# GiulioRomualdi/paper_romualdi_2022_icra_centroidal-mpc-walking

Measured on AMD Instinct MI355X. Metric: centroidal-MPC solves/sec (batch, horizon=20), higher is better.
Workload: dtype f32

## Files before the change

### paper_romualdi_2022_icra_centroidal-mpc-walking_amd/csrc/cmpc_solver.hip

```cpp
#include "cmpc_device.h"
#include "cmpc_launch.h"

#include <cstdlib>
#include <type_traits>
#include <map>
#include <mutex>

#define NS CMPC_NS
#define NF CMPC_NF
#define NQ CMPC_NQ
#define NU CMPC_NU
#define NXA CMPC_NXA
#define NI CMPC_NI
#define PLD 39
#define GLD 30
#define RLD 36
#define NPAN 46
#define GEO 36
#define SQ_TILE_WAVES 6
#define SQ_SPIN_MAX (1 << 20)
#define SQ_PUB_FLOATS (10 * NPAN * 4 + 128 * 4)
#define ZLD 36
#define MSET (NU * RLD + NPAN * RLD + NS * 16)
#define NTRI 256
// ... 16 lines not shown
#define PROF_DECL long long pt_ = __builtin_amdgcn_s_memtime()
#define PROF(slot) do { long long n_ = __builtin_amdgcn_s_memtime(); if (threadIdx.x == 0 && blockIdx.x == 0) g_prof[slot] += n_ - pt_; pt_ = n_; } while (0)
#define PROF2_DECL long long pt2_ = __builtin_amdgcn_s_memtime()
#define PROF3(slot) do { long long n_ = __builtin_amdgcn_s_memtime(); if (threadIdx.x == 192 && blockIdx.x == 0) g_prof[slot] += n_ - pt2_; pt2_ = n_; } while (0)
#define PROF4(slot) do { long long n_ = __builtin_amdgcn_s_memtime(); if (threadIdx.x == 128 && blockIdx.x == 0) g_prof[slot] += n_ - pt2_; pt2_ = n_; } while (0)
#define PROF2(slot) do { long long n_ = __builtin_amdgcn_s_memtime(); if (threadIdx.x == 0 && blockIdx.x == 0) g_prof[slot] += n_ - pt2_; pt2_ = n_; } while (0)
#define PROF5(slot) do { long long n_ = __builtin_amdgcn_s_memtime(); if (threadIdx.x == 216 && blockIdx.x == 0) g_prof[slot] += n_ - pt2_; pt2_ = n_; } while (0)
#define CPROF(i) do { if (ln == 0 && blockIdx.x == 0 && k < N) atomicAdd(reinterpret_cast<unsigned long long*>(&g_prof[32 + 5 * wv + (i)]), (unsigned long long)(__builtin_amdgcn_s_memtime() - pc0_)); } while (0)
#define CPROF2(i) do { if (ln == 0 && blockIdx.x == 0 && k < N) atomicAdd(reinterpret_cast<unsigned long long*>(&g_prof[64 + 8 * wv + (i)]), (unsigned long long)(__builtin_amdgcn_s_memtime() - pc0_)); } while (0)
#ifdef CMPC_PROFILE_LIGHT
#undef PROF2_DECL
#undef PROF2
#undef PROF3
#undef PROF4
#undef PROF5
#undef CPROF
#undef CPROF2
#define CPROF2(i)
#define PROF2_DECL
#define PROF2(slot)
#define PROF3(slot)
#define PROF4(slot)
#define PROF5(slot)
#define CPROF(i)
#define SQPROF_DECL
#define SQPROF(slot)
#else
#define SQPROF_DECL PROF_DECL
#define SQPROF(slot) PROF(slot)
#endif
#else
#define SQPROF_DECL
#define SQPROF(slot)
#define CPROF(i)
#define CPROF2(i)
#define PROF_DECL
#define PROF(slot)
#define PROF2_DECL
#define PROF2(slot)
#define PROF3(slot)
#define PROF4(slot)
#define PROF5(slot)
#endif

struct Ctx {
    CmpcIdx L;
    int N;
    const float* sp;
    float *S, *U, *T, *Z;
    float* LAM;
    float *dS, *dU, *dT, *dZ, *d;
    float *Lf;
    float *geoA;
    float *P0, *Qb, *G, *QuuF, *Pan, *Bval, *Aval, *arow, *ybuf, *fpv, *fpn;
    float *idstrip;
    float *ZT;
    double *QuuD1, *qs1;
    int *Brow, *Arow, *qmask;
    unsigned short* tri;
    double *QuuD, *pv, *pn, *qs, *Pd, *sig, *gco, *redd;
    float* red;
    int* flag;
    int* prog;
};

__device__ inline void wave_lds_sync() { asm volatile("" ::: "memory"); }
typedef __attribute__((address_space(3))) const float* ldsf_t;
typedef __attribute__((address_space(3))) float* ldsw_t;
__device__ inline ldsf_t lds_opaque(const float* p) { ldsf_t q = (ldsf_t)p; asm volatile("" : "+v"(q)); return q; }
__device__ inline ldsw_t lds_opaque_w(float* p) { ldsw_t q = (ldsw_t)p; asm volatile("" : "+v"(q)); return q; }
__device__ inline ldsf_t lds_opaque_again(ldsf_t q) { asm volatile("" : "+v"(q)); return q; }
typedef float v4f __attribute__((ext_vector_type(4)));
typedef float v2f __attribute__((ext_vector_type(2)));
__device__ inline float4 lds_ld4(ldsf_t p)
{
    const v4f v = *reinterpret_cast<__attribute__((address_space(3))) const v4f*>(p);
    return make_float4(v[0], v[1], v[2], v[3]);
}
__device__ inline void lds_ld4x4(ldsf_t p, float4 (&out)[4])
{
    v4f a, b, c, d;
    asm volatile("ds_read_b128 %0, %4\n\tds_read_b128 %1, %4 offset:16\n\tds_read_b128 %2, %4 offset:32\n\tds_read_b128 %3, %4 offset:48\n\ts_waitcnt lgkmcnt(0)"
                 : "=&v"(a), "=&v"(b), "=&v"(c), "=&v"(d)
                 : "v"(p)
                 : "memory");
    out[0] = make_float4(a[0], a[1], a[2], a[3]);
    out[1] = make_float4(b[0], b[1], b[2], b[3]);
    out[2] = make_float4(c[0], c[1], c[2], c[3]);
    out[3] = make_float4(d[0], d[1], d[2], d[3]);
}

typedef unsigned v4u __attribute__((ext_vector_type(4)));
template <bool G>
struct RecRef;
template <>
struct RecRef<false> {
    float* p;
    __device__ RecRef(float* base, int, int k) : p(base + (size_t)REC_N * k) {}
    __device__ float ld(unsigned off) const { return p[off]; }
    __device__ float4 ld4(unsigned off) const { return *reinterpret_cast<const float4*>(p + off); }
    __device__ void st(unsigned off, float v) const { p[off] = v; }
    __device__ void st4(unsigned off, const float4& w) const { *reinterpret_cast<float4*>(p + off) = w; }
};
template <>
struct RecRef<true> {
    typedef __attribute__((address_space(1))) unsigned gu32_t;
    typedef __attribute__((address_space(1))) v4u gv4u_t;
    __amdgpu_buffer_rsrc_t r;
    unsigned so;
    char* gb;
    __device__ RecRef(float* base, int N, int k)
    {
        const unsigned long long a = (unsigned long long)base;
        const unsigned lo = __builtin_amdgcn_readfirstlane((unsigned)a), hi = __builtin_amdgcn_readfirstlane((unsigned)(a >> 32));
// ... 7 lines not shown
        const v4u v = __builtin_amdgcn_raw_buffer_load_b128(r, 4u * off, so, 0);
        return make_float4(__uint_as_float(v.x), __uint_as_float(v.y), __uint_as_float(v.z), __uint_as_float(v.w));
    }
    __device__ void st(unsigned off, float v) const { *(gu32_t*)(gb + 4u * off) = __float_as_uint(v); }
    __device__ void st4(unsigned off, const float4& w) const
    {
        const v4u v = {__float_as_uint(w.x), __float_as_uint(w.y), __float_as_uint(w.z), __float_as_uint(w.w)};
        *(gv4u_t*)(gb + 4u * off) = v;
    }
};

template <bool FG>
__device__ inline void make_ctx(Ctx& c, char* smem, int N, float* fg_base)
{
    constexpr int KBYTES = (sizeof(CmpcConsts) + 15) & ~15;
    c.L.N = N;
    c.N = N;
    double* dp = reinterpret_cast<double*>(smem + KBYTES);
    c.QuuD = dp; dp += 90;
    c.pv = dp; dp += 40; c.pn = dp; dp += 40; c.qs = dp; dp += 16; c.Pd = dp; dp += 40;
    c.sig = dp; dp += NI; c.gco = dp; dp += NI; dp += 2 * NI;
    c.redd = dp; dp += 8;
    c.QuuD1 = c.QuuD; c.qs1 = c.qs;
    if (!FG) { c.QuuD1 = dp; dp += 90; c.qs1 = dp; dp += 16; }
    float* fp = reinterpret_cast<float*>(dp);
    c.QuuF = fp; fp += NU * RLD;
    c.Pan = fp; fp += NPAN * RLD;
    c.ZT = nullptr;
    if (!FG) {
        c.G = nullptr; c.P0 = nullptr;
        c.Qb = fp; fp += NS * 16;
        fp += MSET;
        c.ZT = fp; fp += SQ_PUB_FLOATS;
    } else {
    c.G = fp; fp += (NXA * GLD + 3) & ~3;
    c.P0 = fp; fp += (NXA * PLD + 3) & ~3; c.Qb = fp; fp += NS * 16;
    }
    {
        float* vp = c.QuuF;
        c.dS = vp; vp += NS * (N + 1); c.dU = vp; vp += NU * N; c.dT = vp; vp += NI * N; c.dZ = vp;
    }
    c.ybuf = fp; fp += 96;
    c.idstrip = fp; fp += ID_STRIPS;
    if (!FG) { c.Lf = fp; fp += (size_t)REC_N * N; } else c.Lf = fg_base;
    c.sp = fp; fp += (c.L.np() + 3) & ~3;
    c.S = fp; fp += NS * (N + 1); c.U = fp; fp += NU * N;
    if (!FG || N <= CMPC_TZ_LDS_NMAX) { c.T = fp; fp += NI * N; c.Z = fp; fp += NI * N; }
    else { c.T = fg_base + (size_t)REC_N * N; c.Z = c.T + NI * N; }
    c.d = fp; fp += NS * N;
    c.LAM = fp; fp += NS * (N + 1);
    c.geoA = fp; fp += GEO * N;
    c.Bval = fp; fp += 3 * NU; c.Aval = fp; fp += 3 * NS + 3;
    c.arow = fp; fp += 96 + 12; fp += DSET_F;
    c.fpv = fp; fp += 40; c.fpn = fp; fp += 40; c.red = fp; fp += 24;
    c.Brow = reinterpret_cast<int*>(fp); fp += 3 * NU;
    c.Arow = reinterpret_cast<int*>(fp); fp += 3 * NS + 3; fp += DSET_I;
    c.flag = reinterpret_cast<int*>(fp); fp += 4;
    c.prog = c.flag;
    if (!FG) { c.prog = reinterpret_cast<int*>(fp); fp += 128; }
    c.qmask = reinterpret_cast<int*>(fp); fp += CMPC_NMAX;
    c.tri = reinterpret_cast<unsigned short*>(fp); fp += NTRI / 2;
}

__device__ inline void use_desc_set(Ctx& c, int s)
{
    c.Bval += s * DSET_F; c.Aval += s * DSET_F; c.arow += s * DSET_F;
    c.Brow += s * DSET_I; c.Arow += s * DSET_I;
    c.sig += s * 2 * NI; c.gco += s * 2 * NI;
}

__device__ inline int ub_row(int m) { const int I = m >> 2; return REC_UB + 16 * (8 * I - I * (I - 1) / 2) + (m & 3) * 4 * (8 - I); }
__device__ inline int wt_idx(int j, int a) { return REC_WT + 32 * j + 4 * ((a >> 2) ^ (j & 7)) + (a & 3); }
__device__ inline float half_sum(float v)
{
    const auto r = __builtin_amdgcn_permlane32_swap(__float_as_uint(v), __float_as_uint(v), false, false);
    return __uint_as_float(r[0]) + __uint_as_float(r[1]);
}
__device__ inline float oct_sum(float v)
{
    v += __uint_as_float(__builtin_amdgcn_update_dpp(0u, __float_as_uint(v), 0xB1, 0xF, 0xF, true));
    v += __uint_as_float(__builtin_amdgcn_update_dpp(0u, __float_as_uint(v), 0x4E, 0xF, 0xF, true));
    v += __uint_as_float(__builtin_amdgcn_update_dpp(0u, __float_as_uint(v), 0x141, 0xF, 0xF, true));
    return v;
}
__device__ inline float dot4(const float4& a, const float4& b) { return a.x * b.x + a.y * b.y + a.z * b.z + a.w * b.w; }

__device__ inline float gam_of(const Ctx& c, int ct, int k) { return c.sp[c.L.pGam(ct) + k]; }
__device__ inline float Rm(const float* R, int r, int cc) { return R[3 * cc + r]; }

__device__ inline bool qfree_compute(const Ctx& c, int k, int m)
{
    const int ct = m / 3, i = m % 3;
    const float lo = c.sp[c.L.pLo(ct) + 3 * k + i], hi = c.sp[c.L.pUp(ct) + 3 * k + i];
    return gam_of(c, ct, k) < 0.5f && (hi - lo) > 1e-9f;
}
__device__ inline bool qfree(const Ctx& c, int k, int m) { return (c.qmask[k] >> m) & 1; }
__device__ inline bool outside_subset(const Ctx& c, int ct, int k)
{
    const float g = gam_of(c, ct, k);
    if (g == 0.f) return false;
    if (g != 1.f) return true;
    int kp = -1;
    for (int j = k - 1; j >= 0 && kp < 0; --j) if (gam_of(c, ct, j) < 0.5f) kp = j;
    const float* R = c.sp + c.L.pR(ct) + 9 * k;
    const float* nom = c.sp + c.L.pNom(ct) + 3 * (k + 1);
    const float* lo = c.sp + c.L.pLo(ct) + 3 * k;
    const float* up = c.sp + c.L.pUp(ct) + 3 * k;
// ... 127 lines not shown
}

__device__ inline double grad_sym(const Ctx& c, const CmpcConsts& prm, int k, int m)
{
    const int ct = m / 12, i = m % 3;
    const float* u = c.U + NU * k + 12 * ct;
    const double gam = gam_of(c, ct, k);
    const double mean = 0.25 * ((double)u[i] + (double)u[3 + i] + (double)u[6 + i] + (double)u[9 + i]);
    const double esum = 4.0 * mean * (1.0 - gam);
    const double e = (double)c.U[NU * k + m] - gam * mean;
    return 2.0 * prm.w_sym * (e - 0.25 * gam * esum);
}

__device__ inline float readlane_f(float x, int lane) { return __int_as_float(__builtin_amdgcn_readlane(__float_as_int(x), lane)); }
__device__ inline float uniform_f(float x) { return __int_as_float(__builtin_amdgcn_readfirstlane(__float_as_int(x))); }
__device__ inline double uniform_d(double x)
{
    return __hiloint2double(__builtin_amdgcn_readfirstlane(__double2hiint(x)), __builtin_amdgcn_readfirstlane(__double2loint(x)));
}
__device__ inline double readlane_d(double x, int lane)
{
    const int lo = __builtin_amdgcn_readlane(__double2loint(x), lane);
    const int hi = __builtin_amdgcn_readlane(__double2hiint(x), lane);
    return __hiloint2double(hi, lo);
}

template <int CTRL>
__device__ inline float dpp_f(float v) { return __uint_as_float(__builtin_amdgcn_update_dpp(0u, __float_as_uint(v), CTRL, 0xF, 0xF, true)); }
template <int CTRL>
__device__ inline double dpp_d(double v)
{
    const int lo = __builtin_amdgcn_update_dpp(0, __double2loint(v), CTRL, 0xF, 0xF, true);
    const int hi = __builtin_amdgcn_update_dpp(0, __double2hiint(v), CTRL, 0xF, 0xF, true);
    return __hiloint2double(hi, lo);
}
__device__ inline float amax_nan(float m, float v) { return (v == v) ? fmaxf(m, fabsf(v)) : INFINITY; }
__device__ inline float row_target(float z, float mu_min) { return fmaxf(mu_min * fminf(1.f, z * z), 1e-4f * mu_min); }
__device__ inline float wave_max(float v)
{
    v = fmaxf(v, dpp_f<0xB1>(v));
    v = fmaxf(v, dpp_f<0x4E>(v));
    v = fmaxf(v, dpp_f<0x141>(v));
    v = fmaxf(v, dpp_f<0x140>(v));
    return fmaxf(fmaxf(readlane_f(v, 0), readlane_f(v, 16)), fmaxf(readlane_f(v, 32), readlane_f(v, 48)));
}
__device__ inline double wave_sum(double v)
{
    v += dpp_d<0xB1>(v);
    v += dpp_d<0x4E>(v);
    v += dpp_d<0x141>(v);
    v += dpp_d<0x140>(v);
    return (readlane_d(v, 0) + readlane_d(v, 16)) + (readlane_d(v, 32) + readlane_d(v, 48));
}
template <int NT, int NV>
__device__ inline void block_maxn(float (&v)[NV], float* red, int tid)
{
#pragma unroll
    for (int q = 0; q < NV; ++q) v[q] = wave_max(v[q]);
    __syncthreads();
    if ((tid & 63) == 0) {
#pragma unroll
        for (int q = 0; q < NV; ++q) red[3 * (tid >> 6) + q] = v[q];
    }
    __syncthreads();
#pragma unroll
    for (int q = 0; q < NV; ++q) {
        float r = red[q];
#pragma unroll
        for (int w = 1; w < NT / 64; ++w) r = fmaxf(r, red[3 * w + q]);
        v[q] = uniform_f(r);
    }
}
template <int NT>
__device__ inline double block_sum(double v, double* red, int tid)
{
    v = wave_sum(v);
    __syncthreads();
    if ((tid & 63) == 0) red[tid >> 6] = v;
    __syncthreads();
    double r = red[0];
#pragma unroll
    for (int w = 1; w < NT / 64; ++w) r += red[w];
    return uniform_d(r);
}
template <int NT>
__device__ inline void block_max2_sum(float& m0, float& m1, double& sm, float* red, double* redd, int tid)
{
    m0 = wave_max(m0); m1 = wave_max(m1); sm = wave_sum(sm);
    __syncthreads();
    if ((tid & 63) == 0) { red[3 * (tid >> 6)] = m0; red[3 * (tid >> 6) + 1] = m1; redd[tid >> 6] = sm; }
    __syncthreads();
    float r0 = red[0], r1 = red[1];
    double rs = redd[0];
#pragma unroll
    for (int w = 1; w < NT / 64; ++w) { r0 = fmaxf(r0, red[3 * w]); r1 = fmaxf(r1, red[3 * w + 1]); rs += redd[w]; }
    m0 = uniform_f(r0); m1 = uniform_f(r1); sm = uniform_d(rs);
}

template <int NT>
__device__ inline void all_geo(const Ctx& c, const CmpcConsts& prm, int tid)
{
    for (int e = tid; e < c.N * 24; e += NT) {
        const int k = e / 24, t = e - 24 * k;
        const float* s = c.S + NS * k;
        const int ct = t / 12, j = (t % 12) / 3, i = t % 3;
        const float* R = c.sp + c.L.pR(ct) + 9 * k;
        const float* cn = prm.corners + 12 * ct + 3 * j;
        c.geoA[GEO * k + t] = Rm(R, i, 0) * cn[0] + Rm(R, i, 1) * cn[1] + Rm(R, i, 2) * cn[2] + s[9 + 3 * ct + i] - s[i];
    }
    for (int e = tid; e < c.N * 9; e += NT) {
        const int k = e / 9, t = e - 9 * k, i = t % 3;
        const float* u = c.U + NU * k;
        const float f0 = u[i] + u[3 + i] + u[6 + i] + u[9 + i], f1 = u[12 + i] + u[15 + i] + u[18 + i] + u[21 + i];
        c.geoA[GEO * k + 24 + t] = t < 3 ? f0 : (t < 6 ? f1 : gam_of(c, 0, k) * f0 + gam_of(c, 1, k) * f1);
    }
}

__device__ inline double defect_com(const Ctx& c, const CmpcConsts& prm, int k, int a)
{
    const float* s = c.S + NS * k;
    const float* sn = c.S + NS * (k + 1);
    const double dt = prm.dt;
    return (double)s[a] + dt * (double)s[3 + a] - (double)sn[a];
}
__device__ inline double defect_vel(const Ctx& c, const CmpcConsts& prm, int k, int a)
{
    const float* s = c.S + NS * k;
    const float* u = c.U + NU * k;
    const float* sn = c.S + NS * (k + 1);
    const double dt = prm.dt;
    double acc = (double)c.sp[c.L.pFext() + 3 * k + a] - (a == 2 ? (double)prm.grav : 0.0);
    for (int ct = 0; ct < 2; ++ct) {
        const float* f = u + 12 * ct;
        acc += (double)gam_of(c, ct, k) * ((double)f[a] + (double)f[3 + a] + (double)f[6 + a] + (double)f[9 + a]);
    }
    return (double)s[3 + a] + dt * acc - (double)sn[3 + a];
}
__device__ inline double defect_foot(const Ctx& c, const CmpcConsts& prm, int k, int ct, int a)
{
    const float* s = c.S + NS * k;
    const float* u = c.U + NU * k;
    const float* sn = c.S + NS * (k + 1);
// ... 1779 lines not shown
__device__ void step_lengths(const Ctx& c, int tid, float tau, float& ap, float& ad, int k0 = 0, int k1 = CMPC_NMAX)
{
    float a_p = 1.f, a_d = 1.f;
    const int ke = k1 < c.N ? k1 : c.N;
    for (int e = tid + NI * k0; e < ke * NI; e += NT) {
        const float dt_ = c.dT[e], dz_ = c.dZ[e];
        if (dt_ < 0.f) a_p = fminf(a_p, -tau * c.T[e] / dt_);
        if (dz_ < 0.f) a_d = fminf(a_d, -tau * c.Z[e] / dz_);
    }
    float m[2] = {-a_p, -a_d};
    block_maxn<NT, 2>(m, c.red, tid);
    ap = -m[0]; ad = -m[1];
}

__device__ inline void costate_force_sums(const Ctx& c, int tid, int nth)
{
    const int N = c.N;
    for (int e = tid; e < 9 * N; e += nth) {
        const int k = e / 9, t = e - 9 * k;
        const float* du = c.dU + NU * k;
        const int a = t % 3;
        const float s0 = gam_of(c, 0, k) * (du[a] + du[3 + a] + du[6 + a] + du[9 + a]);
        const float s1 = gam_of(c, 1, k) * (du[12 + a] + du[15 + a] + du[18 + a] + du[21 + a]);
        c.d[NS * k + t] = t < 3 ? s0 : (t < 6 ? s1 : s0 + s1);
    }
}
template <int CTRL>
__device__ inline float dpp_keep(float old, float v) { return __uint_as_float(__builtin_amdgcn_update_dpp(__float_as_uint(old), __float_as_uint(v), CTRL, 0xF, 0xF, false)); }
__device__ inline float lane_next(float v, int lane) { return __int_as_float(__builtin_amdgcn_ds_bpermute(4 * (lane + 1), __float_as_int(v))); }
__device__ inline float suffix_sum(float v, int lane)
{
    v += dpp_f<0x101>(v);
    v += dpp_f<0x102>(v);
    v += dpp_f<0x104>(v);
    v += dpp_f<0x108>(v);
    const float t1 = readlane_f(v, 16), t2 = readlane_f(v, 32), t3 = readlane_f(v, 48);
    const int row = lane >> 4;
    return v + (row == 0 ? t1 + (t2 + t3) : (row == 1 ? t2 + t3 : (row == 2 ? t3 : 0.f)));
}
__device__ inline float suffix_lin(float g, float b, int lane)
{
#define CMPC_LIN_STEP(CT) { const float gn = dpp_keep<CT>(1.f, g), bn = dpp_f<CT>(b); b = fmaf(g, bn, b); g *= gn; }
    CMPC_LIN_STEP(0x101) CMPC_LIN_STEP(0x102) CMPC_LIN_STEP(0x104) CMPC_LIN_STEP(0x108)
#undef CMPC_LIN_STEP
    const int row = lane >> 4;
    const float v48 = readlane_f(b, 48);
    if (row == 2) b = fmaf(g, v48, b);
    const float v32 = readlane_f(b, 32);
    if (row == 1) b = fmaf(g, v32, b);
    const float v16 = readlane_f(b, 16);
    if (row == 0) b = fmaf(g, v16, b);
    return b;
}
template <bool DEFER>
__device__ inline void costate_scan(const Ctx& c, const CmpcConsts& prm, int lane, float ap, bool use_exact, float* vout)
{
    const int N = c.N;
    const bool valid = lane <= N, dyn = lane < N;
    const int k = valid ? lane : N, kd = dyn ? lane : N - 1;
    const float* S = c.S + NS * k;
    const float* dS = c.dS + NS * k;
    const float* geo = c.geoA + GEO * kd;
    const float* dF = c.d + NS * kd;
    const float dtm = dyn ? prm.dt : 0.f;
    const float egm = use_exact ? dtm : 0.f;
    const float on = valid ? 1.f : 0.f;
    float lo[3];
#pragma unroll
    for (int a = 0; a < 3; ++a) lo[a] = c.LAM[NS * (kd + 1) + 6 + a];
    float lold[NS];
    if (!DEFER) {
#pragma unroll
        for (int j = 0; j < NS; ++j) lold[j] = c.LAM[NS * k + j];
    }
    float v[NS];
    float vh1[3];
#pragma unroll
    for (int a = 0; a < 3; ++a) {
        const float b = on * (2.f * prm.w_h) * ((S[6 + a] - c.sp[c.L.pHref() + a + 3 * k]) + dS[6 + a]);
        v[6 + a] = suffix_sum(b, lane);
    }
#pragma unroll
    for (int a = 0; a < 3; ++a) vh1[a] = lane_next(v[6 + a], lane);
#pragma unroll
    for (int a = 0; a < 3; ++a) {
        const int a1 = (a + 1) % 3, a2 = (a + 2) % 3;
        const float w = a == 0 ? 2.f * prm.w_com0 : (a == 1 ? 2.f * prm.w_com1 : prm.wz2[k]);
        float b = w * ((S[a] - c.sp[c.L.pComref() + a + 3 * k]) + dS[a]);
        b += egm * (dF[6 + a2] * lo[a1] - dF[6 + a1] * lo[a2]);
        b += dtm * (vh1[a1] * geo[30 + a2] - vh1[a2] * geo[30 + a1]);
        v[a] = suffix_sum(on * b, lane);
    }
#pragma unroll
    for (int ct = 0; ct < 2; ++ct) {
        const float gam = c.sp[c.L.pGam(ct) + kd];
#pragma unroll
        for (int a = 0; a < 3; ++a) {
            const int a1 = (a + 1) % 3, a2 = (a + 2) % 3, j = 9 + 3 * ct + a;
            float b = (2.f * prm.w_pos) * ((S[j] - c.sp[c.L.pNom(ct) + a + 3 * k]) + dS[j]);
            b += egm * (dF[3 * ct + a1] * lo[a2] - dF[3 * ct + a2] * lo[a1]);
            b -= dtm * gam * (vh1[a1] * geo[24 + 3 * ct + a2] - vh1[a2] * geo[24 + 3 * ct + a1]);
            v[j] = suffix_lin(dyn ? gam : 1.f, on * b, lane);
        }
    }
#pragma unroll
    for (int a = 0; a < 3; ++a) v[3 + a] = suffix_sum(dtm * lane_next(v[a], lane), lane);
    if (valid && lane > 0) {
#pragma unroll
        for (int j = 0; j < NS; ++j) {
            if (DEFER) vout[NS * k + j] = v[j];
            else c.LAM[NS * k + j] = lold[j] + ap * (v[j] - lold[j]);
        }
    }
}

__device__ void costate_update(const Ctx& c, const CmpcConsts& prm, int tid, float ap, bool use_exact)
{
    costate_force_sums(c, tid, blockDim.x);
    __syncthreads();
    if (tid < 64) costate_scan<false>(c, prm, tid, ap, use_exact, nullptr);
    __syncthreads();
}

template <int NT, int NC, bool FG, int PART>
__device__ __attribute__((noinline)) void phase_forward_part(lds_t lds, int Nrt, float* fg_base, bool affine_in)
{
    CMPC_PHASE_PROLOGUE;
    const bool affine = __builtin_amdgcn_readfirstlane((int)affine_in) != 0;
    riccati_forward<NT, NC == 0 ? 1 : (FG ? 2 : SWEEP_UNROLL), FG, PART>(c, prm, tid, affine, 0);
}
template <int NT, int NC, bool FG>
__device__ __forceinline__ void phase_forward_sweep(lds_t lds, int Nrt, float* fg_base, bool affine_in)
{
    if (threadIdx.x < 64) phase_forward_part<NT, NC, FG, 1>(lds, Nrt, fg_base, affine_in);
}
template <int NT, int NC, bool FG>
__device__ __attribute__((noinline)) void phase_forward_tail(lds_t lds, int Nrt, float* fg_base, bool affine_in, int k0_in)
{
    CMPC_PHASE_PROLOGUE;
    const bool affine = __builtin_amdgcn_readfirstlane((int)affine_in) != 0;
    const int k0 = __builtin_amdgcn_readfirstlane(k0_in);
    riccati_forward<NT, 1, FG>(c, prm, tid, affine, k0);
}
template <int NT, int NC, bool FG>
__device__ __attribute__((noinline)) void phase_delta_part(lds_t lds, int Nrt, float* fg_base)
{
    CMPC_PHASE_PROLOGUE;
    riccati_delta<NC == 0 ? 1 : (FG ? 2 : DELTA_UNROLL), FG>(c, prm, tid);
}
template <int NT, int NC, bool FG>
__device__ __forceinline__ void phase_delta(lds_t lds, int Nrt, float* fg_base)
{
    if (threadIdx.x < 64) phase_delta_part<NT, NC, FG>(lds, Nrt, fg_base);
    __syncthreads();
// ... 4 lines not shown
    CMPC_PHASE_PROLOGUE;
    const bool use_exact = __builtin_amdgcn_readfirstlane((int)exact_in) != 0;
    costate_update(c, prm, tid, ap, use_exact);
}
__device__ inline float dual_extrapolate(float z, float dz) { return fmaxf(z + dz, 0.f); }

template <int NT, int NC, bool FG>
__device__ __attribute__((noinline)) void tail_polish(lds_t lds, int Nrt, float* fg_base, int k0_in, bool duals_in)
{
    CMPC_PHASE_PROLOGUE;
    const int k0 = __builtin_amdgcn_readfirstlane(k0_in);
    const bool duals = __builtin_amdgcn_readfirstlane((int)duals_in) != 0;
    bool last = false, blocked = true;
    for (int pi = 0; pi <= prm.tail_iters + 6 && !last; ++pi) {
        last = pi >= prm.tail_iters + 6 || (pi >= prm.tail_iters && !blocked);
        all_geo<NT>(c, prm, tid);
        for (int e = tid + NS * k0; e < NS * N; e += NT) c.d[e] = (float)defect(c, prm, e / NS, e % NS);
        __syncthreads();
        const float cmu = last ? 0.f : -prm.mu_min;
        int fail = riccati_backward<NT, NC, FG>(lds, c, prm, tid, fg_base, prm.exact_hessian != 0, prm.reg, cmu, k0);
        if (fail) {
            __syncthreads();
            fail = riccati_backward<NT, NC, FG>(lds, c, prm, tid, fg_base, false, prm.reg, cmu, k0);
        }
        if (fail) break;
        if (!last) {
            for (int e = tid + NI * k0; e < NI * N; e += NT) c.dZ[e] = row_active(c, e / NI, e % NI) ? row_target(c.Z[e], prm.mu_min) : 0.f;
            __syncthreads();
        }
        phase_forward_tail<NT, NC, FG>(lds, N, fg_base, last, k0);
        float ap, ad;
        step_lengths<NT>(c, tid, last ? 0.999f : 0.99f, ap, ad, k0);
        float bad = 0.f;
        for (int e = tid + NU * k0; e < NU * N; e += NT) bad = amax_nan(bad, c.dU[e]);
        for (int e = tid + NS * (k0 + 1); e < NS * (N + 1); e += NT) bad = amax_nan(bad, c.dS[e]);
        float m1[1] = {bad};
        block_maxn<NT, 1>(m1, c.red, tid);
        if (!(m1[0] < INFINITY)) break;
        blocked = ap < 0.9f || ad < 0.9f;
        for (int e = tid + NS * (k0 + 1); e < NS * (N + 1); e += NT) c.S[e] += ap * c.dS[e];
        for (int e = tid + NU * k0; e < NU * N; e += NT) c.U[e] += ap * c.dU[e];
        if (!last)
            for (int e = tid + NI * k0; e < NI * N; e += NT) { c.T[e] += ap * c.dT[e]; c.Z[e] += ad * c.dZ[e]; }
        else if (duals)
            for (int e = tid + NI * k0; e < NI * N; e += NT) {
                const float tn = c.T[e] + ap * c.dT[e], zn = dual_extrapolate(c.Z[e], c.dZ[e]);
                if (fabsf(tn) < INFINITY && fabsf(zn) < INFINITY) { c.T[e] = tn; c.Z[e] = zn; }
            }
        __syncthreads();
    }
}

struct Resid { float ep, ec, mu; };
template <int NT, int NC, bool FG>
__device__ __attribute__((noinline)) Resid phase_residuals(lds_t lds, int Nrt, float* fg_base, int nrow_in)
{
    CMPC_PHASE_PROLOGUE;
    const int nrow = __builtin_amdgcn_readfirstlane(nrow_in);
    float l_ep = 0.f, l_ec = 0.f, l_chk = 0.f;
    double l_mu = 0.0;
    all_geo<NT>(c, prm, tid);
    for (int e = tid; e < 24 * N; e += NT) {
        const int k = e / 24, r = e - 24 * k, a = r >> 3, cj = r & 7, ct = cj >> 2;
        const int a1 = (a + 1) % 3, a2 = (a + 2) % 3;
        const float* s = c.S + NS * k;
        const float* f = c.U + NU * k + 3 * cj;
        const float* R = c.sp + c.L.pR(ct) + 9 * k;
        const float* cn = prm.corners + 3 * cj;
        const double r1 = (double)Rm(R, a1, 0) * cn[0] + (double)Rm(R, a1, 1) * cn[1] + (double)Rm(R, a1, 2) * cn[2] + (double)s[9 + 3 * ct + a1] - (double)s[a1];
        const double r2 = (double)Rm(R, a2, 0) * cn[0] + (double)Rm(R, a2, 1) * cn[1] + (double)Rm(R, a2, 2) * cn[2] + (double)s[9 + 3 * ct + a2] - (double)s[a2];
        double t = (double)gam_of(c, ct, k) * (r1 * (double)f[a2] - r2 * (double)f[a1]);
        t += dpp_d<0xB1>(t);
        t += dpp_d<0x4E>(t);
        t += dpp_d<0x141>(t);
        if (cj == 0) {
            const double dv = (double)s[6 + a] + (double)prm.dt * ((double)c.sp[c.L.pText() + 3 * k + a] + t) - (double)c.S[NS * (k + 1) + 6 + a];
            c.d[NS * k + 6 + a] = (float)dv;
            l_ep = fmaxf(l_ep, fabsf((float)dv));
            l_chk += (float)dv;
        }
    }
    constexpr int LGRP = (3 * NC + 63) / 64 * 64;
    if constexpr (NC > 0 && !FG && 4 * LGRP <= NT) {
        static_assert((LGRP & (LGRP - 1)) == 0, "the lane inside a group is taken with a mask");
        const int tl = tid - (NT - 4 * LGRP);
        const int grp = __builtin_amdgcn_readfirstlane(tl >= 0 ? tl / LGRP : -1);
        const int l = tl & (LGRP - 1);
        if (grp >= 0 && l < 3 * NC) {
            const int a = (l >= NC ? 1 : 0) + (l >= 2 * NC ? 1 : 0), k = l - NC * a;
            double dv;
            int i;
            if (grp == 0) { i = a; dv = defect_com(c, prm, k, a); }
            else if (grp == 1) { i = 3 + a; dv = defect_vel(c, prm, k, a); }
            else { i = 9 + 3 * (grp - 2) + a; dv = defect_foot(c, prm, k, grp - 2, a); }
            c.d[NS * k + i] = (float)dv;
            l_ep = fmaxf(l_ep, fabsf((float)dv));
            l_chk += (float)dv;
        }
    } else {
        for (int e = tid; e < 12 * N; e += NT) {
            const int k = e / 12, ii = e - 12 * k, i = ii < 6 ? ii : ii + 3;
            const double dv = ii < 3 ? defect_com(c, prm, k, ii) : (ii < 6 ? defect_vel(c, prm, k, ii - 3) : defect_foot(c, prm, k, ii < 9 ? 0 : 1, ii < 9 ? ii - 6 : ii - 9));
            c.d[NS * k + i] = (float)dv;
            l_ep = fmaxf(l_ep, fabsf((float)dv));
            l_chk += (float)dv;
        }
    }
    if constexpr (NC > 0) {
        for_slots<0, RowSlots<NT, NC>::R>([&](auto qc) {
            constexpr int q = decltype(qc)::value;
            int e;
            float val, dot;
            const int st = row_slot<NT, NC, q, false>(c, prm, tid, e, val, dot);
            const float t = c.T[e], z = c.Z[e];
            if (st & 2) {
                const float rv = val + t;
                l_ep = fmaxf(l_ep, fabsf(rv));
                l_ec = fmaxf(l_ec, t * z);
                l_chk += rv + t * z;
                l_mu += (double)t * z;
            }
        });
    } else {
        for (int e = tid; e < NI * N; e += NT) {
            const int k = e / NI, i = e % NI;
            if (row_active(c, k, i)) {
                const float t = c.T[e], z = c.Z[e];
                const float rv = row_val(c, prm, k, i, c.U + NU * k) + t;
                l_ep = fmaxf(l_ep, fabsf(rv));
                l_ec = fmaxf(l_ec, t * z);
                l_chk += rv + t * z;
                l_mu += (double)t * z;
            }
        }
    }
    if (!(fabsf(l_chk) < INFINITY)) l_ep = INFINITY;
    block_max2_sum<NT>(l_ep, l_ec, l_mu, c.red, c.redd, tid);
    Resid r;
    r.ep = l_ep; r.ec = l_ec; r.mu = (float)(l_mu / (double)nrow);
    return r;
}

template <int NT, int NC, bool FG>
__device__ __attribute__((noinline)) float phase_update(lds_t lds, int Nrt, float* fg_base, float ap_in, float ad_in)
{
    CMPC_PHASE_PROLOGUE;
    const float ap = uniform_f(ap_in), ad = uniform_f(ad_in);
    for (int e = tid; e < NS * (N + 1); e += NT) c.S[e] += ap * c.dS[e];
    for (int e = tid; e < NU * N; e += NT) c.U[e] += ap * c.dU[e];
    for (int e = tid; e < NI * N; e += NT) {
        const float tn = c.T[e] + ap * c.dT[e];
        float zn = c.Z[e] + ad * c.dZ[e];
        c.T[e] = tn; c.Z[e] = zn;
    }
    float l_st = 0.f, l_sf = 0.f, l_fm = 1.f, l_chk2 = 0.f;
    for (int e = tid; e < NS * (N + 1); e += NT) { const float ds = c.dS[e]; l_st = fmaxf(l_st, fabsf(ds)); l_chk2 += ds; }
    for (int e = tid; e < NU * N; e += NT) {
        const int k = e / NU, m = e % NU;
        const float du = c.dU[e];
        l_chk2 += du;
        if (m < NF) {
            const float* f = c.dU + NU * k + 12 * (m / 12) + m % 3;
            const float mean = 0.25f * (f[0] + f[3] + f[6] + f[9]);
            l_sf = fmaxf(l_sf, fabsf(du - gam_of(c, m / 12, k) * mean));
            if (k > 0) l_sf = fmaxf(l_sf, fabsf(du - c.dU[e - NU]));
            l_fm = fmaxf(l_fm, fabsf(c.U[e]));
        } else l_st = fmaxf(l_st, fabsf(du));
    }
    if (!(fabsf(l_chk2) < INFINITY)) l_st = INFINITY;
    float m3[3] = {l_st, l_sf, l_fm};
    block_maxn<NT, 3>(m3, c.red, tid);
    return ap * fmaxf(m3[0], m3[1] / m3[2]);
}

template <int NT, int NC, bool FG>
__device__ __attribute__((noinline)) bool phase_finish(lds_t lds, int Nrt, float* fg_base, bool duals_in)
{
    CMPC_PHASE_PROLOGUE;
    const bool duals = __builtin_amdgcn_readfirstlane((int)duals_in) != 0;
    float ap, ad;
    step_lengths<NT>(c, tid, 0.999f, ap, ad);
    const int kt = N - prm.tail_stages;
    float l_all = 0.f, l_tail = 0.f, l_fm = 1.f;
    for (int e = tid; e < NS * (N + 1); e += NT) l_all = amax_nan(l_all, c.dS[e]);
    for (int e = tid; e < NU * N; e += NT) {
        const float du = c.dU[e];
        l_all = amax_nan(l_all, du);
        if (e % NU < NF) {
            l_fm = fmaxf(l_fm, fabsf(c.U[e]));
            if (e >= NU * kt) l_tail = fmaxf(l_tail, fabsf(du));
// ... 148 lines not shown
    step_lengths<NT>(c, tid, uniform_f(tau), r.ap, r.ad);
    return r;
}

struct Centre { float sigma, mu_t; };
template <int NT, int NC, bool FG>
__device__ __attribute__((noinline)) Centre phase_corrector_targets(lds_t lds, int Nrt, float* fg_base, float ap_in, float ad_in, float mu_in, int nrow_in)
{
    CMPC_PHASE_PROLOGUE;
    const float ap = uniform_f(ap_in), ad = uniform_f(ad_in), mu_cur = uniform_f(mu_in);
    const int nrow = __builtin_amdgcn_readfirstlane(nrow_in);
    double l_aff = 0.0;
    for (int e = tid; e < NI * N; e += NT)
        if (row_active(c, e / NI, e % NI)) l_aff += (double)(c.T[e] + ap * c.dT[e]) * (double)(c.Z[e] + ad * c.dZ[e]);
    const float mu_aff = (float)(block_sum<NT>(l_aff, c.redd, tid) / (double)nrow);
    Centre r;
    r.sigma = mu_aff / mu_cur;
    r.sigma = r.sigma * r.sigma * r.sigma;
    r.mu_t = fmaxf(fmaxf(r.sigma, prm.sigma_min) * mu_cur, prm.mu_min);
    for (int e = tid; e < NI * N; e += NT) {
        const float cmu = row_active(c, e / NI, e % NI) ? r.mu_t - c.dT[e] * c.dZ[e] : 0.f;
        c.dZ[e] = cmu;
        c.dT[e] = cmu / c.T[e];
    }
    __syncthreads();
    return r;
}

template <int NT, int NC, bool FG>
__device__ __attribute__((noinline)) Centre phase_affine_post(lds_t lds, int Nrt, float* fg_base, float mu_in, int nrow_in)
{
    CMPC_PHASE_PROLOGUE;
    typedef RowSlots<NT, NC> RS;
    constexpr int R = RS::R;
    const float mu_cur = uniform_f(mu_in);
    const int nrow = __builtin_amdgcn_readfirstlane(nrow_in);
    __syncthreads();
    float t[R], z[R], dt[R], dz[R];
    int ei[R], st[R];
    float a_p = 1.f, a_d = 1.f;
    for_slots<0, R>([&](auto qc) {
        constexpr int q = decltype(qc)::value;
        float val, dot;
        st[q] = row_slot<NT, NC, q, true>(c, prm, tid, ei[q], val, dot);
        t[q] = c.T[ei[q]]; z[q] = c.Z[ei[q]];
        const float r = val + t[q];
        dt[q] = -r - dot;
        dz[q] = (0.f - z[q] * t[q]) / t[q] - (z[q] / t[q]) * dt[q];
        if (st[q] & 2) {
            if (dt[q] < 0.f) a_p = fminf(a_p, -t[q] / dt[q]);
            if (dz[q] < 0.f) a_d = fminf(a_d, -z[q] / dz[q]);
        }
    });
    float m[2] = {-a_p, -a_d};
    block_maxn<NT, 2>(m, c.red, tid);
    const float ap = -m[0], ad = -m[1];
    double l_aff = 0.0;
#pragma unroll
    for (int q = 0; q < R; ++q)
        if (st[q] & 2) l_aff += (double)(t[q] + ap * dt[q]) * (double)(z[q] + ad * dz[q]);
    const float mu_aff = (float)(block_sum<NT>(l_aff, c.redd, tid) / (double)nrow);
    Centre r;
    r.sigma = mu_aff / mu_cur;
    r.sigma = r.sigma * r.sigma * r.sigma;
    r.mu_t = fmaxf(fmaxf(r.sigma, prm.sigma_min) * mu_cur, prm.mu_min);
#pragma unroll
    for (int q = 0; q < R; ++q) {
        if (st[q] & 1) {
            const float cmu = (st[q] & 2) ? r.mu_t - dt[q] * dz[q] : 0.f;
            c.dZ[ei[q]] = cmu;
            c.dT[ei[q]] = (st[q] & 2) ? cmu / t[q] : 0.f;
        }
    }
    __syncthreads();
    return r;
}

struct FinalStep { float ap, ad, step; };
template <int NT, int NC, bool FG>
__device__ __attribute__((noinline)) FinalStep phase_final_post(lds_t lds, int Nrt, float* fg_base, float tau_in, bool exact_in)
{
    CMPC_PHASE_PROLOGUE;
    constexpr int NTR = NT - 64;
    typedef RowSlots<NTR, NC> RS;
    constexpr int R = RS::R;
    const float tau = uniform_f(tau_in);
    const bool use_exact = __builtin_amdgcn_readfirstlane((int)exact_in) != 0;
    float* vbuf = c.dT;
    __syncthreads();
    float t[R], z[R], dt[R], dz[R];
    int ei[R], st[R];
    float a_p = 1.f, a_d = 1.f;
    if (tid < 64) {
        costate_force_sums(c, tid, 64);
        wave_lds_sync();
        costate_scan<true>(c, prm, tid, 0.f, use_exact, vbuf);
#pragma unroll
        for (int q = 0; q < R; ++q) { t[q] = 1.f; z[q] = 0.f; dt[q] = 0.f; dz[q] = 0.f; ei[q] = 0; st[q] = 0; }
    } else {
        for_slots<0, R>([&](auto qc) {
            constexpr int q = decltype(qc)::value;
            float val, dot;
            st[q] = row_slot<NTR, NC, q, true>(c, prm, tid - 64, ei[q], val, dot);
            t[q] = c.T[ei[q]]; z[q] = c.Z[ei[q]];
            const float cmu = c.dZ[ei[q]];
            const float r = val + t[q];
            dt[q] = -r - dot;
            dz[q] = (cmu - z[q] * t[q]) / t[q] - (z[q] / t[q]) * dt[q];
            if (st[q] & 2) {
                if (dt[q] < 0.f) a_p = fminf(a_p, -tau * t[q] / dt[q]);
                if (dz[q] < 0.f) a_d = fminf(a_d, -tau * z[q] / dz[q]);
            }
        });
    }
    float m[2] = {-a_p, -a_d};
    block_maxn<NT, 2>(m, c.red, tid);
    const float ap = -m[0], ad = -m[1];
#pragma unroll
    for (int q = 0; q < R; ++q)
        if (st[q] & 2) {
            c.T[ei[q]] = t[q] + ap * dt[q];
            c.Z[ei[q]] = z[q] + ad * dz[q];
        }
    for (int e = tid; e < NS * (N + 1); e += NT) {
        const float lold = c.LAM[e];
        c.LAM[e] = lold + ap * (vbuf[e] - lold);
        c.S[e] += ap * c.dS[e];
    }
    for (int e = tid; e < NU * N; e += NT) c.U[e] += ap * c.dU[e];
    float l_st = 0.f, l_sf = 0.f, l_fm = 1.f, l_chk2 = 0.f;
    for (int e = tid; e < NS * (N + 1); e += NT) { const float ds = c.dS[e]; l_st = fmaxf(l_st, fabsf(ds)); l_chk2 += ds; }
    for (int e = tid; e < NU * N; e += NT) {
        const int k = e / NU, mm = e % NU;
        const float du = c.dU[e];
        l_chk2 += du;
        if (mm < NF) {
            const float* f = c.dU + NU * k + 12 * (mm / 12) + mm % 3;
            const float mean = 0.25f * (f[0] + f[3] + f[6] + f[9]);
            l_sf = fmaxf(l_sf, fabsf(du - gam_of(c, mm / 12, k) * mean));
            if (k > 0) l_sf = fmaxf(l_sf, fabsf(du - c.dU[e - NU]));
            l_fm = fmaxf(l_fm, fabsf(c.U[e]));
        } else l_st = fmaxf(l_st, fabsf(du));
    }
    if (!(fabsf(l_chk2) < INFINITY)) l_st = INFINITY;
    float m3[3] = {l_st, l_sf, l_fm};
    block_maxn<NT, 3>(m3, c.red, tid);
    FinalStep r;
    r.ap = ap; r.ad = ad; r.step = ap * fmaxf(m3[0], m3[1] / m3[2]);
    return r;
}

template <int NT, int NC, bool FG>
__device__ __attribute__((noinline)) void phase_export(lds_t lds, int Nrt, float* fg_base, float* x, float* dq, int status_in)
{
    CMPC_PHASE_PROLOGUE;
    for (int e = tid; e < NS * (N + 1); e += NT) {
        const int k = e / NS, i = e % NS;
        if (i < 9) x[c.L.oCom() + 3 * (N + 1) * (i / 3) + 3 * k + i % 3] = c.S[e];
        else x[c.L.oPos((i - 9) / 3) + 3 * k + (i - 9) % 3] = c.S[e];
    }
    for (int e = tid; e < NU * N; e += NT) {
        const int k = e / NU, m = e % NU;
        if (m < NF) x[c.L.oF(m / 12, (m % 12) / 3) + 3 * k + m % 3] = c.U[e];
        else {
            const int q = m - 24, ct = q / 3, i = q % 3;
            const float v = gam_of(c, ct, k) < 0.5f ? (c.S[NS * (k + 1) + 9 + q] - c.S[NS * k + 9 + q]) / prm.dt : 0.f;
            x[c.L.oVel(ct) + 3 * k + i] = v;
        }
    }
    if (dq) {
        const int status = __builtin_amdgcn_readfirstlane(status_in);
        __syncthreads();
        if (status != 3) {
            all_geo<NT>(c, prm, tid);
            for (int e = tid; e < NS * (N + 1); e += NT) c.dS[e] = 0.f;
            for (int e = tid; e < NS * N; e += NT) c.d[e] = 0.f;
            __syncthreads();
            if (tid < 64) costate_scan<true>(c, prm, tid, 0.f, false, c.LAM);
            __syncthreads();
        }
        for (int e = tid; e < NS * (N + 1); e += NT) dq[e] = e < NS ? (e == 0 ? (float)status : 0.f) : c.LAM[e];
        for (int e = tid; e < NI * N; e += NT) { dq[NS * (N + 1) + e] = c.T[e]; dq[NS * (N + 1) + NI * N + e] = c.Z[e]; }
    }
#ifdef CMPC_PROFILE
    if (prm.hwid_probe) {
        __syncthreads();
        if ((threadIdx.x & 63) == 0) x[threadIdx.x >> 6] = (float)(__builtin_amdgcn_s_getreg((31 << 11) | 4) & 0xffff);
    }
#endif
}

template <int NT, int NC, bool FG>
__global__ __launch_bounds__(NT, FG ? 3 : 1) void cmpc_solve_kernel(CmpcParams kp)
{
    extern __shared__ __attribute__((aligned(16))) char smem[];
    const int b = blockIdx.x;
    if (kp.ended && kp.ended[b] >= 0) return;
    const bool fresh = kp.start && kp.start[b] == kp.tick;
    const bool warm = kp.warm && !fresh;
// ... 224 lines not shown
```

Measured before the change: 372,100.

## Split costate scan across three waves per axis and drop leading reduction barriers

For the 512-thread non-FG configuration, the final-post phase now runs the costate scan as three waves, one per spatial axis, instead of a single wave. The remaining waves handle the row slots, so fewer threads do row work. Leading __syncthreads in block reductions are skipped in several lean passes, and a second reduction buffer (red1) replaces the unused fpn slot so that back-to-back reductions do not race. The change risks missing syncs if any earlier shared-memory use conflicts, and it duplicates some per-axis work such as recomputing the vh suffix sums in each wave.

```diff
diff --git a/paper_romualdi_2022_icra_centroidal-mpc-walking_amd/csrc/cmpc_solver.hip b/paper_romualdi_2022_icra_centroidal-mpc-walking_amd/csrc/cmpc_solver.hip
--- a/paper_romualdi_2022_icra_centroidal-mpc-walking_amd/csrc/cmpc_solver.hip
+++ b/paper_romualdi_2022_icra_centroidal-mpc-walking_amd/csrc/cmpc_solver.hip
@@ -92,14 +92,14 @@
     float *dS, *dU, *dT, *dZ, *d;
     float *Lf;
     float *geoA;
-    float *P0, *Qb, *G, *QuuF, *Pan, *Bval, *Aval, *arow, *ybuf, *fpv, *fpn;
+    float *P0, *Qb, *G, *QuuF, *Pan, *Bval, *Aval, *arow, *ybuf, *fpv;
     float *idstrip;
     float *ZT;
     double *QuuD1, *qs1;
     int *Brow, *Arow, *qmask;
     unsigned short* tri;
     double *QuuD, *pv, *pn, *qs, *Pd, *sig, *gco, *redd;
-    float* red;
+    float *red, *red1;
     int* flag;
     int* prog;
 };
@@ -213,7 +213,7 @@
     c.geoA = fp; fp += GEO * N;
     c.Bval = fp; fp += 3 * NU; c.Aval = fp; fp += 3 * NS + 3;
     c.arow = fp; fp += 96 + 12; fp += DSET_F;
-    c.fpv = fp; fp += 40; c.fpn = fp; fp += 40; c.red = fp; fp += 24;
+    c.fpv = fp; fp += 40; c.red1 = fp; fp += 40; c.red = fp; fp += 24;
     c.Brow = reinterpret_cast<int*>(fp); fp += 3 * NU;
     c.Arow = reinterpret_cast<int*>(fp); fp += 3 * NS + 3; fp += DSET_I;
     c.flag = reinterpret_cast<int*>(fp); fp += 4;
@@ -447,12 +447,12 @@
     v += dpp_d<0x140>(v);
     return (readlane_d(v, 0) + readlane_d(v, 16)) + (readlane_d(v, 32) + readlane_d(v, 48));
 }
-template <int NT, int NV>
+template <int NT, int NV, bool LEAD = true>
 __device__ inline void block_maxn(float (&v)[NV], float* red, int tid)
 {
 #pragma unroll
     for (int q = 0; q < NV; ++q) v[q] = wave_max(v[q]);
-    __syncthreads();
+    if (LEAD) __syncthreads();
     if ((tid & 63) == 0) {
 #pragma unroll
         for (int q = 0; q < NV; ++q) red[3 * (tid >> 6) + q] = v[q];
@@ -466,11 +466,11 @@
         v[q] = uniform_f(r);
     }
 }
-template <int NT>
+template <int NT, bool LEAD = true>
 __device__ inline double block_sum(double v, double* red, int tid)
 {
     v = wave_sum(v);
-    __syncthreads();
+    if (LEAD) __syncthreads();
     if ((tid & 63) == 0) red[tid >> 6] = v;
     __syncthreads();
     double r = red[0];
@@ -478,11 +478,11 @@
     for (int w = 1; w < NT / 64; ++w) r += red[w];
     return uniform_d(r);
 }
-template <int NT>
+template <int NT, bool LEAD = true>
 __device__ inline void block_max2_sum(float& m0, float& m1, double& sm, float* red, double* redd, int tid)
 {
     m0 = wave_max(m0); m1 = wave_max(m1); sm = wave_sum(sm);
-    __syncthreads();
+    if (LEAD) __syncthreads();
     if ((tid & 63) == 0) { red[3 * (tid >> 6)] = m0; red[3 * (tid >> 6) + 1] = m1; redd[tid >> 6] = sm; }
     __syncthreads();
     float r0 = red[0], r1 = red[1];
@@ -2368,6 +2368,73 @@
     if (row == 0) b = fmaf(g, v16, b);
     return b;
 }
+__device__ __forceinline__ float costate_com_b(float w, float err, float egm, float dtm, float dF1, float dF2, float lo1, float lo2, float vh1, float vh2, float g1,
+                                               float g2)
+{
+    float b = w * err;
+    b += egm * (dF2 * lo1 - dF1 * lo2);
+    b += dtm * (vh1 * g2 - vh2 * g1);
+    return b;
+}
+__device__ __forceinline__ float costate_foot_b(float w, float err, float egm, float dtm, float gam, float dF1, float dF2, float lo1, float lo2, float vh1, float vh2,
+                                                float g1, float g2)
+{
+    float b = w * err;
+    b += egm * (dF1 * lo2 - dF2 * lo1);
+    b -= dtm * gam * (vh1 * g2 - vh2 * g1);
+    return b;
+}
+__device__ __forceinline__ float sel3(const float (&v)[3], int i) { return i == 0 ? v[0] : (i == 1 ? v[1] : v[2]); }
+__device__ inline void costate_scan_axis(const Ctx& c, const CmpcConsts& prm, int lane, int ax, bool use_exact, float* vout)
+{
+    const int N = c.N;
+    const bool valid = lane <= N, dyn = lane < N;
+    const int k = valid ? lane : N, kd = dyn ? lane : N - 1;
+    const int a1 = ax == 2 ? 0 : ax + 1, a2 = ax == 0 ? 2 : ax - 1;
+    const float* S = c.S + NS * k;
+    const float* dS = c.dS + NS * k;
+    const float* geo = c.geoA + GEO * kd;
+    const float* du = c.dU + NU * kd;
+    const float* lo = c.LAM + NS * (kd + 1) + 6;
+    const float dtm = dyn ? prm.dt : 0.f;
+    const float egm = use_exact ? dtm : 0.f;
+    const float on = valid ? 1.f : 0.f;
+    const float gam0 = gam_of(c, 0, kd), gam1 = gam_of(c, 1, kd);
+    float dF1[3], dF2[3];
+    dF1[0] = gam0 * (du[a1] + du[3 + a1] + du[6 + a1] + du[9 + a1]);
+    dF1[1] = gam1 * (du[12 + a1] + du[15 + a1] + du[18 + a1] + du[21 + a1]);
+    dF1[2] = dF1[0] + dF1[1];
+    dF2[0] = gam0 * (du[a2] + du[3 + a2] + du[6 + a2] + du[9 + a2]);
+    dF2[1] = gam1 * (du[12 + a2] + du[15 + a2] + du[18 + a2] + du[21 + a2]);
+    dF2[2] = dF2[0] + dF2[1];
+    const float lo1 = lo[a1], lo2 = lo[a2];
+    float vh[3], vhn[3];
+#pragma unroll
+    for (int a = 0; a < 3; ++a) {
+        const float b = on * (2.f * prm.w_h) * ((S[6 + a] - c.sp[c.L.pHref() + a + 3 * k]) + dS[6 + a]);
+        vh[a] = suffix_sum(b, lane);
+    }
+#pragma unroll
+    for (int a = 0; a < 3; ++a) vhn[a] = lane_next(vh[a], lane);
+    const float vh1 = sel3(vhn, a1), vh2 = sel3(vhn, a2);
+    const float w = ax == 0 ? 2.f * prm.w_com0 : (ax == 1 ? 2.f * prm.w_com1 : prm.wz2[k]);
+    const float bc = costate_com_b(w, (S[ax] - c.sp[c.L.pComref() + ax + 3 * k]) + dS[ax], egm, dtm, dF1[2], dF2[2], lo1, lo2, vh1, vh2, geo[30 + a1], geo[30 + a2]);
+    const float vc = suffix_sum(on * bc, lane);
+    float vf[2];
+#pragma unroll
+    for (int ct = 0; ct < 2; ++ct) {
+        const float gam = ct ? gam1 : gam0;
+        const int j = 9 + 3 * ct + ax;
+        const float b = costate_foot_b(2.f * prm.w_pos, (S[j] - c.sp[c.L.pNom(ct) + ax + 3 * k]) + dS[j], egm, dtm, gam, dF1[ct], dF2[ct], lo1, lo2, vh1, vh2,
+                                       geo[24 + 3 * ct + a1], geo[24 + 3 * ct + a2]);
+        vf[ct] = suffix_lin(dyn ? gam : 1.f, on * b, lane);
+    }
+    const float vv = suffix_sum(dtm * lane_next(vc, lane), lane);
+    if (valid && lane > 0) {
+        float* o = vout + NS * k + ax;
+        o[0] = vc; o[3] = vv; o[6] = sel3(vh, ax); o[9] = vf[0]; o[12] = vf[1];
+    }
+}
 template <bool DEFER>
 __device__ inline void costate_scan(const Ctx& c, const CmpcConsts& prm, int lane, float ap, bool use_exact, float* vout)
 {
@@ -2402,9 +2469,8 @@
     for (int a = 0; a < 3; ++a) {
         const int a1 = (a + 1) % 3, a2 = (a + 2) % 3;
         const float w = a == 0 ? 2.f * prm.w_com0 : (a == 1 ? 2.f * prm.w_com1 : prm.wz2[k]);
-        float b = w * ((S[a] - c.sp[c.L.pComref() + a + 3 * k]) + dS[a]);
-        b += egm * (dF[6 + a2] * lo[a1] - dF[6 + a1] * lo[a2]);
-        b += dtm * (vh1[a1] * geo[30 + a2] - vh1[a2] * geo[30 + a1]);
+        const float b = costate_com_b(w, (S[a] - c.sp[c.L.pComref() + a + 3 * k]) + dS[a], egm, dtm, dF[6 + a1], dF[6 + a2], lo[a1], lo[a2], vh1[a1], vh1[a2],
+                                      geo[30 + a1], geo[30 + a2]);
         v[a] = suffix_sum(on * b, lane);
     }
 #pragma unroll
@@ -2413,9 +2479,8 @@
 #pragma unroll
         for (int a = 0; a < 3; ++a) {
             const int a1 = (a + 1) % 3, a2 = (a + 2) % 3, j = 9 + 3 * ct + a;
-            float b = (2.f * prm.w_pos) * ((S[j] - c.sp[c.L.pNom(ct) + a + 3 * k]) + dS[j]);
-            b += egm * (dF[3 * ct + a1] * lo[a2] - dF[3 * ct + a2] * lo[a1]);
-            b -= dtm * gam * (vh1[a1] * geo[24 + 3 * ct + a2] - vh1[a2] * geo[24 + 3 * ct + a1]);
+            const float b = costate_foot_b(2.f * prm.w_pos, (S[j] - c.sp[c.L.pNom(ct) + a + 3 * k]) + dS[j], egm, dtm, gam, dF[3 * ct + a1], dF[3 * ct + a2], lo[a1],
+                                           lo[a2], vh1[a1], vh1[a2], geo[24 + 3 * ct + a1], geo[24 + 3 * ct + a2]);
             v[j] = suffix_lin(dyn ? gam : 1.f, on * b, lane);
         }
     }
@@ -2526,6 +2591,8 @@
 }
 
 struct Resid { float ep, ec, mu; };
+template <int NT, int NC, bool FG>
+constexpr bool kLeanPasses = NT == 512 && NC > 0 && !FG;
 template <int NT, int NC, bool FG>
 __device__ __attribute__((noinline)) Resid phase_residuals(lds_t lds, int Nrt, float* fg_base, int nrow_in)
 {
@@ -2609,7 +2676,7 @@
         }
     }
     if (!(fabsf(l_chk) < INFINITY)) l_ep = INFINITY;
-    block_max2_sum<NT>(l_ep, l_ec, l_mu, c.red, c.redd, tid);
+    block_max2_sum<NT, !kLeanPasses<NT, NC, FG>>(l_ep, l_ec, l_mu, c.red, c.redd, tid);
     Resid r;
     r.ep = l_ep; r.ec = l_ec; r.mu = (float)(l_mu / (double)nrow);
     return r;
@@ -2864,14 +2931,15 @@
             if (dz[q] < 0.f) a_d = fminf(a_d, -z[q] / dz[q]);
         }
     });
+    constexpr bool LEAD = !kLeanPasses<NT, NC, FG>;
     float m[2] = {-a_p, -a_d};
-    block_maxn<NT, 2>(m, c.red, tid);
+    block_maxn<NT, 2, LEAD>(m, c.red, tid);
     const float ap = -m[0], ad = -m[1];
     double l_aff = 0.0;
 #pragma unroll
     for (int q = 0; q < R; ++q)
         if (st[q] & 2) l_aff += (double)(t[q] + ap * dt[q]) * (double)(z[q] + ad * dz[q]);
-    const float mu_aff = (float)(block_sum<NT>(l_aff, c.redd, tid) / (double)nrow);
+    const float mu_aff = (float)(block_sum<NT, LEAD>(l_aff, c.redd, tid) / (double)nrow);
     Centre r;
     r.sigma = mu_aff / mu_cur;
     r.sigma = r.sigma * r.sigma * r.sigma;
@@ -2893,7 +2961,9 @@
 __device__ __attribute__((noinline)) FinalStep phase_final_post(lds_t lds, int Nrt, float* fg_base, float tau_in, bool exact_in)
 {
     CMPC_PHASE_PROLOGUE;
-    constexpr int NTR = NT - 64;
+    constexpr bool LEAN = kLeanPasses<NT, NC, FG>;
+    constexpr int NCW = LEAN ? 3 : 1;
+    constexpr int NTR = NT - 64 * NCW;
     typedef RowSlots<NTR, NC> RS;
     constexpr int R = RS::R;
     const float tau = uniform_f(tau_in);
@@ -2903,17 +2973,20 @@
     float t[R], z[R], dt[R], dz[R];
     int ei[R], st[R];
     float a_p = 1.f, a_d = 1.f;
-    if (tid < 64) {
-        costate_force_sums(c, tid, 64);
-        wave_lds_sync();
-        costate_scan<true>(c, prm, tid, 0.f, use_exact, vbuf);
+    if (tid < 64 * NCW) {
+        if constexpr (LEAN) costate_scan_axis(c, prm, tid & 63, __builtin_amdgcn_readfirstlane(tid >> 6), use_exact, vbuf);
+        else {
+            costate_force_sums(c, tid, 64);
+            wave_lds_sync();
+            costate_scan<true>(c, prm, tid, 0.f, use_exact, vbuf);
+        }
 #pragma unroll
         for (int q = 0; q < R; ++q) { t[q] = 1.f; z[q] = 0.f; dt[q] = 0.f; dz[q] = 0.f; ei[q] = 0; st[q] = 0; }
     } else {
         for_slots<0, R>([&](auto qc) {
             constexpr int q = decltype(qc)::value;
             float val, dot;
-            st[q] = row_slot<NTR, NC, q, true>(c, prm, tid - 64, ei[q], val, dot);
+            st[q] = row_slot<NTR, NC, q, true>(c, prm, tid - 64 * NCW, ei[q], val, dot);
             t[q] = c.T[ei[q]]; z[q] = c.Z[ei[q]];
             const float cmu = c.dZ[ei[q]];
             const float r = val + t[q];
@@ -2926,7 +2999,7 @@
         });
     }
     float m[2] = {-a_p, -a_d};
-    block_maxn<NT, 2>(m, c.red, tid);
+    block_maxn<NT, 2, !LEAN>(m, c.red, tid);
     const float ap = -m[0], ad = -m[1];
 #pragma unroll
     for (int q = 0; q < R; ++q)
@@ -2956,7 +3029,7 @@
     }
     if (!(fabsf(l_chk2) < INFINITY)) l_st = INFINITY;
     float m3[3] = {l_st, l_sf, l_fm};
-    block_maxn<NT, 3>(m3, c.red, tid);
+    block_maxn<NT, 3, !LEAN>(m3, LEAN ? c.red1 : c.red, tid);
     FinalStep r;
     r.ap = ap; r.ad = ad; r.step = ap * fmaxf(m3[0], m3[1] / m3[2]);
     return r;
```

Measured after the change: 378,300, median of 6. 1.7% higher.
